# terry19850829Home/kafkastreams-cep

Hardware: AMD Instinct MI355X
Metric: events/sec (whole node), 3-stage A->B->C over 1M keys; achieved HBM GB/s (higher is better)
Workload: dtype int32; 1 GPU; C2: 3-stage strict A->B->C, processor mode; events_per_gpu=100000000, keys_per_gpu=1000000, matches_per_gpu=1531088, matches_total=1531088, parallelism=1 GPU, kernels=built-in, nfa_kernel=auto

## Files before the change

kafkastreams-cep_amd/csrc/abi.cpp:

```cpp
#include <dlfcn.h>
#include <hip/hip_runtime.h>
#include <string.h>

#include <algorithm>
#include <atomic>
#include <chrono>
#include <memory>
#include <string>
#include <vector>

#include "../../include/kcep.h"
#include "build_id.h"
#include "kcep_internal.h"
#include "jit.h"

namespace kcep {
hipError_t stencil_launch(const StencilLaunch& L, hipEvent_t ev0, hipEvent_t ev1, hipStream_t st);
int64_t stencil_tiles(int64_t n);
hipError_t stencil_post(const int32_t* key, const int32_t* out, int k, int64_t nm, int32_t* mkey,
                        const StencilProgram* P, unsigned long long* sum, hipStream_t st);
hipError_t stencil_resolve_launch(const int32_t* key, const int32_t* out, int k, int64_t nm, const StencilCarry& C,
                                  int64_t* pos, const StencilProgram* P, unsigned long long* sum, hipStream_t st);
hipError_t stencil_deliver_launch(const int32_t* key, const int32_t* out, int k, const int64_t* total, int64_t out_cap,
                                  const StencilCarry& C, int64_t host_cap, int64_t* hdr, int32_t* hkey, int64_t* hpos,
// ... 274 lines not shown
      if (arrs[i].src && arrs[i].bytes) {
        memcpy(h + at[size_t(i)], arrs[i].src, arrs[i].bytes);
        *arrs[i].dst = static_cast<uint8_t*>(dptr) + at[size_t(i)];
      }
    s->zc_slot = j;
    return CEP_OK;
  }
  bool pinned = true;
  for (int i = 0; i < na && pinned; i++)
    if (arrs[i].src && arrs[i].bytes) pinned = host_pinned(arrs[i].src);
  if (s->dstage.ensure(total)) return fail(CEP_E_HIP, "staging allocation failed");
  uint8_t* dev = s->dstage.as<uint8_t>();
  for (int i = 0; i < na; i++)
    if (arrs[i].src && arrs[i].bytes) *arrs[i].dst = dev + at[size_t(i)];
  if (pinned) {
    for (int i = 0; i < na; i++)
      if (arrs[i].src && arrs[i].bytes)
        HIPCHECK(hipMemcpyAsync(dev + at[size_t(i)], arrs[i].src, arrs[i].bytes, hipMemcpyHostToDevice, st));
    if (!s->h2d_ev) HIPCHECK(hipEventCreateWithFlags(&s->h2d_ev, hipEventDisableTiming));
    HIPCHECK(hipEventRecord(s->h2d_ev, st));
    s->h2d_wait = true;
    return CEP_OK;
  }
  const size_t chunk = std::min(total, size_t(2) << 20);
  for (size_t c0 = 0; c0 < total; c0 += chunk) {
    const size_t c1 = std::min(total, c0 + chunk);
    const int j = s->ring_next;
    s->ring_next ^= 1;
    if (s->ring_ev[j]) HIPCHECK(hipEventSynchronize(s->ring_ev[j]));
    else HIPCHECK(hipEventCreateWithFlags(&s->ring_ev[j], hipEventDisableTiming));
    const size_t want = std::min(total, chunk);
    if (s->ring_cap[j] < want) {
      if (s->ring[j]) HIPCHECK(hipHostFree(s->ring[j]));
      s->ring[j] = nullptr;
      s->ring_cap[j] = 0;
      HIPCHECK(hipHostMalloc(&s->ring[j], want, hipHostMallocMapped));
      s->ring_cap[j] = want;
    }
    uint8_t* h = static_cast<uint8_t*>(s->ring[j]);
    for (int i = 0; i < na; i++) {
      if (!arrs[i].src || !arrs[i].bytes) continue;
      const size_t a = std::max(c0, at[size_t(i)]), b = std::min(c1, at[size_t(i)] + arrs[i].bytes);
      if (a < b) memcpy(h + (a - c0), static_cast<const uint8_t*>(arrs[i].src) + (a - at[size_t(i)]), b - a);
    }
    HIPCHECK(hipMemcpyAsync(dev + c0, h, c1 - c0, hipMemcpyHostToDevice, st));
    HIPCHECK(hipEventRecord(s->ring_ev[j], st));
  }
  return CEP_OK;
}

void dl_layout(const cep_session* s, int slot, int64_t*& hdr, int32_t*& hkey, int64_t*& hpos) {
  hdr = static_cast<int64_t*>(s->dl[slot]);
  hkey = reinterpret_cast<int32_t*>(hdr + 4);
  hpos = hdr + 4 + (s->dl_cap + 1) / 2 + 1;
}

int push_stencil(cep_session* s, const cep_batch* b, hipStream_t st) {
  const StencilProgram& SP = s->pat->prog.stencil;
  const void* col = b->n_cols ? b->cols[SP.col] : nullptr;
  const int32_t* key = b->key_id;
  const int32_t* topic = SP.use_topic ? b->topic : nullptr;
  const size_t vs = type_size(SP.coltype);
  if (b->mem == CEP_MEM_HOST && b->n > 0) {
    HostArr arrs[3] = {{key, size_t(b->n) * 4, reinterpret_cast<const void**>(&key)},
                       {col, size_t(b->n) * vs, &col},
                       {topic, size_t(b->n) * 4, reinterpret_cast<const void**>(&topic)}};
    int rc = stage_host(s, arrs, SP.use_topic ? 3 : 2, st, true);
    if (rc) return rc;
  }
  if (SP.use_topic && !topic && b->n > 0) {
    if (s->h_topic.ensure(size_t(b->n) * 4)) return fail(CEP_E_HIP, "staging allocation failed");
    HIPCHECK(hipMemsetAsync(s->h_topic.p, 0, size_t(b->n) * 4, st));
    topic = s->h_topic.as<int32_t>();
  }
  if ((reinterpret_cast<uintptr_t>(key) | reinterpret_cast<uintptr_t>(col) | reinterpret_cast<uintptr_t>(topic)) & 15)
    return fail(CEP_E_ARG, "device columns must be 16-byte aligned");
  s->d_key = key;
  int64_t* tc = s->status.as<int64_t>();
  const int64_t ntiles = stencil_tiles(b->n);
  StencilLaunch L{key, col, topic, b->n, s->prog.as<StencilProgram>(), SP.k, SP.coltype, SP.use_topic, SP.chain,
                  s->slots.as<int32_t>(), tc, tc + ntiles + 1, s->counter.as<int64_t>(), s->out.as<int32_t>(),
                  s->out_cap, s->total.as<int64_t>(), StencilCarry{}, !getenv_flag("KCEP_STENCIL_KEYED"), nullptr};
  L.key_mode = getenv_flag("KCEP_STENCIL_SPARSE_KEYS") ? 1 : getenv_flag("KCEP_STENCIL_DENSE_KEYS") ? 2 : 0;
  if (s->carry) {
    L.clear_flag = s->hflags.as<unsigned long long>() + (s->halo_stamp & 1);
    L.carry = StencilCarry{s->halo.as<HaloHdr>(), s->hpos.as<int64_t>(), SP.k - 1, ++s->halo_stamp,
                           int32_t(std::min<int64_t>(s->opts.max_keys, INT32_MAX)), s->base,
                           s->hflags.as<unsigned long long>() + (s->halo_stamp & 1), s->cur_pos,
                           s->cur_pos ? 1 : 0};
    s->last_gpos = s->cur_pos;
    s->halo_base = s->base;
    s->base += b->n;
  }
  if (s->carry && (b->flags & CEP_BATCH_DELIVER)) {
    const int k = SP.k;
    const int64_t host_cap = std::min<int64_t>(s->out_cap, int64_t(1) << 20);
    if (!s->dl[0]) {
      const size_t bytes = 8 * (4 + size_t(host_cap + 1) / 2 + 1) + size_t(host_cap) * size_t(k) * 8;
      for (int j = 0; j < 2; j++) {
        HIPCHECK(hipHostMalloc(&s->dl[j], bytes, hipHostMallocMapped | hipHostMallocCoherent));
        memset(s->dl[j], 0, 32);
      }
      s->dl_cap = host_cap;
      if (s->dl_ticket.ensure(16)) return fail(CEP_E_HIP, "allocation failed");
      HIPCHECK(hipMemsetAsync(s->dl_ticket.p, 0, 16, st));
    }
    if (s->out_cap > host_cap &&
        (s->mkey.ensure(size_t(s->out_cap) * 4) || s->opos.ensure(size_t(s->out_cap) * size_t(k) * 8)))
      return fail(CEP_E_HIP, "allocation failed");
    const int slot = int((s->dl_stamp + 1) & 1);
    dl_layout(s, slot, L.deliver.hdr, L.deliver.hkey, L.deliver.hpos);
    s->dl_pid[slot] = s->push_id;
    L.deliver.dkey = s->mkey.as<int32_t>();
    L.deliver.dpos = s->opos.as<int64_t>();
    L.deliver.host_cap = s->dl_cap;
    L.deliver.ticket = s->dl_ticket.as<unsigned>();
    L.deliver.stamp = ++s->dl_stamp;
    if (s->cur_pos && b->n > 0) {
      if (s->a_moff.ensure(size_t(b->n) * 8) || s->a_tmp.ensure(size_t(b->n / 1024 + 4) * 8) || s->scal.ensure(64))
        return fail(CEP_E_HIP, "allocation failed");
      L.deliver.a_cnt = s->a_cnt.as<int64_t>();
      L.deliver.a_head = s->a_head.as<int32_t>();
      L.deliver.a_moff = s->a_moff.as<int64_t>();
      L.deliver.a_tot = s->scal.as<int64_t>() + 6;
      L.deliver.a_tmp = s->a_tmp.as<int64_t>();
      L.deliver.a_n = b->n;
    }
    s->delivered = true;
  }
  HIPCHECK(stencil_launch(L, s->timing ? s->ev0 : nullptr, s->timing ? s->ev1 : nullptr, st));
  if (s->timing) HIPCHECK(hipEventRecord(s->eb1, st));
  return CEP_OK;
}

int64_t read_i64(const void* dev, hipStream_t st, int* rc) {
  int64_t v = 0;
  if (hipMemcpyAsync(&v, dev, sizeof v, hipMemcpyDeviceToHost, st) != hipSuccess ||
      hipStreamSynchronize(st) != hipSuccess)
    *rc = CEP_E_HIP;
  return v;
}

int carry_gc(cep_session* s, int64_t min_words, hipStream_t st) {
  const int64_t nk = s->opts.max_keys;
  int rc = CEP_OK;
  if (s->flag.ensure(size_t(nk) * 8) || s->idx.ensure(size_t(nk) * 8) ||
      s->scan_tmp.ensure(size_t(nk / 1024 + 2) * 8) || s->scal.ensure(64))
    return fail(CEP_E_HIP, "allocation failed");
  int64_t* scal = s->scal.as<int64_t>();
  HIPCHECK(carry_sizes_launch(s->ctab.as<int64_t>(), nk, s->cpool.as<int32_t>(), s->flag.as<int64_t>(), st));
  HIPCHECK(exclusive_scan(s->flag.as<int64_t>(), nk, s->idx.as<int64_t>(), scal + 5, s->scan_tmp.as<int64_t>(), st));
  const int64_t live = read_i64(scal + 5, st, &rc);
  if (rc) return fail(rc, "carry size");
  const int64_t cap = std::max<int64_t>({2 * live, min_words, int64_t(1) << 20});
  DBuf fresh;
  if (fresh.ensure(size_t(cap) * 4)) return fail(CEP_E_RUN_CAPACITY, "cannot allocate the carried-state pool");
  HIPCHECK(carry_move_launch(s->ctab.as<int64_t>(), nk, s->cpool.as<int32_t>(), s->idx.as<int64_t>(),
                             fresh.as<int32_t>(), st));
  HIPCHECK(hipStreamSynchronize(st));
  s->cpool.release();
  s->cpool = fresh;
  fresh.p = nullptr;
  s->cpool_words = cap;
  s->cpool_used = live;
  return CEP_OK;
}
// ... 1924 lines not shown
```

kafkastreams-cep_amd/csrc/kcep_internal.h:

```cpp
#pragma once
#include <hip/hip_runtime_api.h>
#include <stdint.h>
#include "kcep_dev.h"

#include <memory>
#include <string>
#include <vector>

namespace kcep {

struct Expr {
  uint8_t op = 0, t = 0, ct = 0;
  int32_t i32 = 0;
  int64_t i64 = 0;
  double f64 = 0;
  int col = 0, name = 0;
  std::string sname;
  std::shared_ptr<Expr> a, b;
};
using ExprP = std::shared_ptr<Expr>;

struct Fold {
  int state;
  uint8_t type;
// ... 101 lines not shown
KCEP_HD inline int64_t halo_gpos(const StencilCarry& C, int64_t r) { return C.gpos ? C.gpos[r] : C.base + r; }
KCEP_HD inline int halo_old(const HaloHdr& h, int32_t stamp) {
  const int32_t a = h.stamp[0] < stamp ? h.stamp[0] : -1, b = h.stamp[1] < stamp ? h.stamp[1] : -1;
  return a >= b ? 0 : 1;
}

struct DeliverArgs {
  int64_t* hdr = nullptr;
  int32_t* hkey = nullptr;
  int64_t* hpos = nullptr;
  int32_t* dkey = nullptr;
  int64_t* dpos = nullptr;
  int64_t host_cap = 0;
  unsigned* ticket = nullptr;
  int64_t stamp = 0;
  int64_t* a_cnt = nullptr;
  int32_t* a_head = nullptr;
  int64_t* a_moff = nullptr;
  int64_t* a_tot = nullptr;
  int64_t* a_tmp = nullptr;
  int64_t a_n = 0;
};
struct GroupArgs {
  const int32_t* key;
  int32_t* g_key;
  int32_t* arr;
  int64_t* pos;
  int64_t base;
  const uint8_t* valid; uint8_t* g_valid;
  const int32_t* topic; int32_t* g_topic;
  const int32_t* partition; int32_t* g_partition;
  const int64_t* offset; int64_t* g_offset;
  const int64_t* ts; int64_t* g_ts;
  const void* cols[16]; void* g_cols[16];
  int32_t coltype[16];
  int32_t ncols;
  int64_t* cnt;
  int64_t* ecnt;
  int32_t max_keys;
  uint32_t stamp;
  unsigned long long* head;
  int32_t* node_top;
  int32_t *node_key, *node_chunk, *node_cnt, *node_next, *node_prefix, *node_leader, *rec_node, *rec_rank;
  int64_t* start;
  unsigned long long* cursor;
};
hipError_t group_launch(const GroupArgs& G, int64_t n, hipStream_t st);
hipError_t arrival_reorder(const int64_t* mrec, const int32_t* mkey, const int64_t* eoff, const int32_t* ename,
                           const int64_t* erec, int64_t nm, int64_t ne, int64_t base, int64_t n, int64_t* cnt,
                           int64_t* ecnt, int32_t* head, int64_t* moff, int64_t* moff_e, int64_t* tot, int64_t* tmp,
                           int64_t* o_rec, int32_t* o_key, int64_t* o_eoff, int32_t* o_name, int64_t* o_erec,
                           hipStream_t st);
hipError_t stencil_arrival_ranks(const int32_t* out, int k, const int64_t* total, int64_t out_cap, const int64_t* gpos,
                                 int64_t base, int64_t n, int64_t* cnt, int32_t* head, int64_t* moff, int64_t* tot,
                                 int64_t* tmp, hipStream_t st);
#ifndef KCEP_ST_DENSE
#define KCEP_ST_DENSE 512
#endif
constexpr int ST_DENSE = KCEP_ST_DENSE;
constexpr int ST_DENSE_KEYED = 1024;
#ifndef ST_KEYED_DENSE
#define ST_KEYED_DENSE 0
#endif

struct StencilLaunch {
  const int32_t* key;
  const void* val;
  const int32_t* topic;
  int64_t n;
  const StencilProgram* prog_dev;
  int k, coltype, use_topic, chain;
  int32_t* slots;
  int64_t* tile_count;
  int64_t* tile_pre;
  int64_t* scan_tmp;
  int32_t* out;
  int64_t out_cap;
  int64_t* total;
  StencilCarry carry;
  int plain;
  unsigned long long* clear_flag;
  DeliverArgs deliver;
  int key_mode = 0;
};

int lower_general(Program& P, std::string& why);
bool wave_stateful(const DevProgram& D);
int compile_ir(const uint8_t* ir, size_t len, Program& out, std::string& err);

struct RcIn {
  const int64_t* pos;
  const int32_t* key;
  const int32_t* topic;
  const int32_t* partition;
  const int64_t* offset;
  const int64_t* ts;
  const void* cols[16];
};
struct RcExt {
  int32_t *key, *topic, *partition, *seg;
  int64_t *offset, *ts, *pos;
  void* cols[16];
  int32_t coltype[16];
  int32_t ncols;
  int64_t cap;
};
hipError_t runs_carry_build(const RcIn& B, int64_t n, int64_t base, const int64_t* seg_flag, const int64_t* seg_idx,
                            const int64_t* seg_start, const int64_t* nseg, const int64_t* rtab, const int64_t* rpool,
                            int64_t* tlen, int64_t* toff, int64_t* total, int64_t* scan_tmp, const RcExt& X,
                            hipStream_t st, bool lens_only, int32_t max_keys);
hipError_t runs_carry_count(int64_t* out, int64_t nb, const int64_t* tails, int64_t cap, hipStream_t st);
hipError_t runs_carry_tails(const RcExt& X, int64_t ext_n, int64_t n, const int64_t* nseg, const int64_t* seg_start,
                            const int32_t* key, const int64_t* toff, const int32_t* end_of, unsigned long long* tstart,
                            int64_t* newlen, int64_t* noff, int64_t* new_total, int64_t* scan_tmp, int64_t* top,
                            int64_t* rpool, int64_t* rtab, hipStream_t st, const int64_t* ext_n_dev, const int64_t* bad);
hipError_t runs_carry_gc(int64_t* rtab, int64_t nkeys, int RW, const int64_t* src, int64_t* dst, int64_t* len,
                         int64_t* off, int64_t* total, int64_t* scan_tmp, hipStream_t st);

}
```

kafkastreams-cep_amd/csrc/stencil.hip:

```cpp
#include "stencil_kernel.h"

namespace kcep {

hipError_t stencil_count_k1(const StencilLaunch& L, hipStream_t st);
hipError_t stencil_count_k2(const StencilLaunch& L, hipStream_t st);
hipError_t stencil_count_k3(const StencilLaunch& L, hipStream_t st);
hipError_t stencil_count_k4(const StencilLaunch& L, hipStream_t st);
hipError_t stencil_count_k5(const StencilLaunch& L, hipStream_t st);
hipError_t stencil_count_k6(const StencilLaunch& L, hipStream_t st);
hipError_t stencil_count_k7(const StencilLaunch& L, hipStream_t st);
hipError_t stencil_count_k8(const StencilLaunch& L, hipStream_t st);

struct SlotFormat {
  int k, plain, chain, carry, dense, kdense;
  int64_t nsuper;
  int sub;
  __device__ __forceinline__ void load(const int32_t* slots, int64_t t, int64_t c, int64_t m, int32_t& v,
                                       uint32_t& a) const {
    a = 0;
    if (dense) {
      v = m < ST_DENSE ? slots[t * ST_DENSE + m] : slots[nsuper * ST_DENSE + t * int64_t(sub) * ST_TILE + m];
      return;
    }
    if (kdense && c <= ST_DENSE_KEYED) {
// ... 145 lines not shown
                                                  int64_t* __restrict__ total, unsigned long long* __restrict__ clear_flag) {
  __shared__ int64_t s_w[16];
  const int tid = threadIdx.x, lane = tid & 63, wid = tid >> 6;
  const int64_t per = (nt + 1023) / 1024, a = tid * per, b = a + per < nt ? a + per : nt;
  int64_t sum = 0;
  int64_t r8[8];
  const bool one_pass = per <= 8;
  if (one_pass) {
#pragma unroll
    for (int i = 0; i < 8; i++) { r8[i] = a + i < b ? cnt[a + i] : 0; sum += r8[i]; }
  } else {
    for (int64_t c = a; c < b; c += 8) {
      int64_t v[8];
#pragma unroll
      for (int i = 0; i < 8; i++) v[i] = c + i < b ? cnt[c + i] : 0;
#pragma unroll
      for (int i = 0; i < 8; i++) sum += v[i];
    }
  }
  int64_t incl = sum;
#pragma unroll
  for (int d = 1; d < 64; d <<= 1) {
    const int64_t y = __shfl_up(incl, d, 64);
    if (lane >= d) incl += y;
  }
  if (lane == 63) s_w[wid] = incl;
  __syncthreads();
  int64_t run = incl - sum;
  for (int w = 0; w < wid; w++) run += s_w[w];
  if (one_pass) {
#pragma unroll
    for (int i = 0; i < 8; i++)
      if (a + i < b) { pre[a + i] = run; run += r8[i]; }
  } else {
    for (int64_t c = a; c < b; c += 8) {
      int64_t v[8];
#pragma unroll
      for (int i = 0; i < 8; i++) v[i] = c + i < b ? cnt[c + i] : 0;
#pragma unroll
      for (int i = 0; i < 8; i++) {
        if (c + i < b) pre[c + i] = run;
        run += v[i];
      }
    }
  }
  if (tid == 1023) *total = run;
  if (tid == 0 && clear_flag) *clear_flag = 0;
}

constexpr int SMALL_FINISH = 1024;
__global__ __launch_bounds__(1024) void stencil_finish_small(const int32_t* __restrict__ slots,
                                                             const int64_t* __restrict__ cnt, int64_t nt, int k,
                                                             int32_t* __restrict__ out, int64_t out_cap, int sub,
                                                             int64_t* __restrict__ total,
                                                             unsigned long long* __restrict__ clear_flag,
                                                             SlotFormat F) {
  __shared__ int64_t s_pre[SMALL_FINISH + 1];
  __shared__ int64_t s_w[16];
  const int tid = threadIdx.x, lane = tid & 63, wid = tid >> 6;
  const int64_t c = tid < nt ? cnt[tid] : 0;
  int64_t incl = c;
#pragma unroll
  for (int d = 1; d < 64; d <<= 1) {
    const int64_t y = __shfl_up(incl, d, 64);
    if (lane >= d) incl += y;
  }
  if (lane == 63) s_w[wid] = incl;
  __syncthreads();
  int64_t run = incl - c;
  for (int w = 0; w < wid; w++) run += s_w[w];
  s_pre[tid] = run;
  if (tid == 1023) { s_pre[SMALL_FINISH] = run + c; *total = run + c; }
  if (tid == 0 && clear_flag) *clear_flag = 0;
  __syncthreads();
  for (int64_t t = wid; t < nt; t += 16) {
    const int64_t pre = s_pre[t], m = s_pre[t + 1] - pre;
    if (pre + m > out_cap) continue;
    int32_t* dst = out + pre * k;
    for (int64_t q = lane; q < m; q += 64) {
      int32_t v;
      uint32_t a;
      F.load(slots, t, m, q, v, a);
      for (int s2 = 0; s2 < k; s2++) dst[q * k + s2] = F.value(v, a, s2);
    }
  }
}

__device__ __forceinline__ void deliver_done(unsigned* ticket, unsigned nblocks, int64_t* hdr, int64_t stamp) {
  __syncthreads();
  if (threadIdx.x == 0) {
    __threadfence_system();
    const unsigned prev = atomicAdd(ticket, 1u);
    if (prev == nblocks - 1) {
      __threadfence_system();
      *ticket = 0;
      *reinterpret_cast<volatile int64_t*>(hdr + 2) = stamp;
    }
  }
}

__global__ __launch_bounds__(256) void stencil_finish_deliver(const int32_t* __restrict__ slots,
                                                              const int64_t* __restrict__ cnt, int64_t nt, int k,
                                                              int32_t* __restrict__ out, int64_t out_cap, int sub,
                                                              int64_t* __restrict__ total,
                                                              unsigned long long* __restrict__ clear_flag,
                                                              SlotFormat F, const int32_t* __restrict__ key,
                                                              StencilCarry C, int64_t host_cap, int64_t* __restrict__ hdr,
                                                              int32_t* __restrict__ hkey, int64_t* __restrict__ hpos,
                                                              int32_t* __restrict__ dkey, int64_t* __restrict__ dpos,
                                                              unsigned* ticket, int64_t stamp) {
  __shared__ int64_t s_red[2][4];
  const int64_t t = blockIdx.x;
  const int lane = threadIdx.x & 63, wid = threadIdx.x >> 6;
  int64_t before = 0, all = 0;
  for (int64_t i = threadIdx.x; i < nt; i += 256) {
    const int64_t c = cnt[i];
    all += c;
    if (i < t) before += c;
  }
#pragma unroll
  for (int d = 32; d >= 1; d >>= 1) {
    before += __shfl_xor(before, d, 64);
    all += __shfl_xor(all, d, 64);
  }
  if (lane == 0) { s_red[0][wid] = before; s_red[1][wid] = all; }
  __syncthreads();
  const int64_t pre = s_red[0][0] + s_red[0][1] + s_red[0][2] + s_red[0][3];
  const int64_t tot = s_red[1][0] + s_red[1][1] + s_red[1][2] + s_red[1][3];
  if (t == 0 && threadIdx.x == 0) {
    *total = tot;
    hdr[0] = tot;
    hdr[1] = int64_t(*C.flags);
    if (clear_flag) *clear_flag = 0;
  }
  const int64_t m = cnt[t];
  if (pre + m <= out_cap) {
    for (int64_t q = threadIdx.x; q < m; q += 256) {
      const int64_t i = pre + q;
      int32_t row[STENCIL_MAX_K], last = 0, v;
      uint32_t av;
      F.load(slots, t, m, q, v, av);
#pragma unroll
      for (int s = 0; s < STENCIL_MAX_K; s++)
        if (s < k) {
          row[s] = F.value(v, av, s);
          out[i * k + s] = row[s];
          last = row[s];
        }
      const int32_t kk = key[last];
      const bool kok = kk >= 0 && kk < C.max_keys;
      const HaloHdr* h = kok ? C.hdr + kk : nullptr;
      const int old = kok ? halo_old(*h, C.stamp) : 0;
      const int64_t* hp = kok ? C.pos + (2 * int64_t(kk) + old) * C.km1 : nullptr;
      const bool host = i < host_cap;
      int64_t* p = host ? hpos + i * k : dpos + i * k;
#pragma unroll
      for (int s = 0; s < STENCIL_MAX_K; s++)
        if (s < k) {
          const int32_t r = row[s];
          p[s] = r >= 0 ? halo_gpos(C, r) : (r == -1 || !kok ? -1 : hp[h->cnt[old] - (-r - 1)]);
        }
      if (host) hkey[i] = kk;
      else dkey[i] = kk;
    }
  }
  deliver_done(ticket, unsigned(gridDim.x), hdr, stamp);
// ... 105 lines not shown
      int64_t j = s_tpre[a >> 6];
      for (int64_t b = (a & ~int64_t(63)) >> 2; b < (a >> 2); b++) {
        const uint32_t w = s_cnt[b];
        j += (w & 0xFF) + ((w >> 8) & 0xFF) + ((w >> 16) & 0xFF) + (w >> 24);
      }
      for (int64_t b = a & ~int64_t(3); b < a; b++) j += (s_cnt[b >> 2] >> (8 * (b & 3))) & 0xFF;
      if (F.chain)
        for (int64_t p = q - 1; p >= 0 && F.entry(slots, t, m, p, k - 1) == last; p--) j++;
      const bool kok = kk >= 0 && kk < C.max_keys;
      const HaloHdr* h = kok ? C.hdr + kk : nullptr;
      const int old = kok ? halo_old(*h, C.stamp) : 0;
      const int64_t* hp = kok ? C.pos + (2 * int64_t(kk) + old) * C.km1 : nullptr;
      const bool host = j < host_cap;
      int64_t* pp = host ? hpos + j * k : dpos + j * k;
#pragma unroll
      for (int s2 = 0; s2 < STENCIL_MAX_K; s2++)
        if (s2 < k) {
          const int32_t r = row[s2];
          pp[s2] = r >= 0 ? halo_gpos(C, r) : (r == -1 || !kok ? -1 : hp[h->cnt[old] - (-r - 1)]);
        }
      if (host) hkey[j] = kk;
      else dkey[j] = kk;
    }
  }
  (void)n;
  deliver_done(ticket, 1u, hdr, stamp);
}

static hipError_t stencil_count(const StencilLaunch& L, hipStream_t st) {
  if (L.chain && L.k != 3 && L.k != 4) return hipErrorInvalidValue;
  switch (L.k) {
    case 1: return stencil_count_k1(L, st);
    case 2: return stencil_count_k2(L, st);
    case 3: return stencil_count_k3(L, st);
    case 4: return stencil_count_k4(L, st);
    case 5: return stencil_count_k5(L, st);
    case 6: return stencil_count_k6(L, st);
    case 7: return stencil_count_k7(L, st);
    case 8: return stencil_count_k8(L, st);
  }
  return hipErrorInvalidValue;
}

hipError_t exclusive_scan(const int64_t* in, int64_t n, int64_t* out, int64_t* total, int64_t* tmp, hipStream_t st);
hipError_t stencil_deliver_launch(const int32_t* key, const int32_t* out, int k, const int64_t* total, int64_t out_cap,
                                  const StencilCarry& C, const DeliverArgs& D, hipStream_t st);

hipError_t stencil_launch(const StencilLaunch& L, hipEvent_t ev0, hipEvent_t ev1, hipStream_t st) {
  const DeliverArgs& D = L.deliver;
  if (L.n <= 0) {
    hipError_t e = ev0 ? hipEventRecord(ev0, st) : hipSuccess;
    if (e == hipSuccess && L.clear_flag) e = hipMemsetAsync(L.clear_flag, 0, 8, st);
    if (e == hipSuccess && ev1) e = hipEventRecord(ev1, st);
    if (e == hipSuccess) e = hipMemsetAsync(L.total, 0, sizeof(int64_t), st);
    if (e == hipSuccess && D.hdr)
      e = stencil_deliver_launch(L.key, L.out, L.k, L.total, 0, L.carry, D, st);
    return e;
  }
  const int64_t ntiles = (L.n + ST_TILE - 1) / ST_TILE;
  const int sub = stencil_sub(ntiles);
  const int64_t nsuper = (ntiles + sub - 1) / sub;
  hipError_t e = ev0 ? hipEventRecord(ev0, st) : hipSuccess;
  if (e == hipSuccess) e = stencil_count(L, st);
  if (e == hipSuccess && ev1) e = hipEventRecord(ev1, st);
  if (e != hipSuccess) return e;
  const bool plain = L.plain && !L.chain && L.k <= 7;
  const SlotFormat F{L.k, plain, L.chain, L.carry.hdr != nullptr, plain && !L.carry.hdr && ST_PLAIN_STAGE,
                     !plain && !L.carry.hdr && ST_KEYED_DENSE, nsuper, sub};
  if (nsuper <= SMALL_FINISH && D.hdr && L.carry.hdr && D.a_moff && L.n <= ARR_SMALL) {
    hipLaunchKernelGGL(stencil_finish_deliver_arrival, dim3(1), dim3(1024), 0, st, L.slots, L.tile_count, nsuper, L.k,
                       L.out, L.out_cap, sub, L.total, L.clear_flag, F, L.key, L.carry, L.n, D.host_cap, D.hdr, D.hkey,
                       D.hpos, D.dkey, D.dpos, D.ticket, D.stamp);
    return hipGetLastError();
  }
  if (nsuper <= SMALL_FINISH && D.hdr && L.carry.hdr && !D.a_moff) {
    hipLaunchKernelGGL(stencil_finish_deliver, dim3(unsigned(nsuper)), dim3(256), 0, st, L.slots, L.tile_count, nsuper,
                       L.k, L.out, L.out_cap, sub, L.total, L.clear_flag, F, L.key, L.carry, D.host_cap, D.hdr, D.hkey,
                       D.hpos, D.dkey, D.dpos, D.ticket, D.stamp);
    return hipGetLastError();
  }
  if (nsuper <= SMALL_FINISH) {
    hipLaunchKernelGGL(stencil_finish_small, dim3(1), dim3(1024), 0, st, L.slots, L.tile_count, nsuper, L.k, L.out,
                       L.out_cap, sub, L.total, L.clear_flag, F);
  } else {
    if (nsuper <= 8 * 1024) {
      hipLaunchKernelGGL(tile_scan, dim3(1), dim3(1024), 0, st, L.tile_count, nsuper, L.tile_pre, L.total, L.clear_flag);
    } else {
      hipError_t e = exclusive_scan(L.tile_count, nsuper, L.tile_pre, L.total, L.scan_tmp, st);
      if (e == hipSuccess && L.clear_flag) e = hipMemsetAsync(L.clear_flag, 0, 8, st);
      if (e != hipSuccess) return e;
    }
    if (F.dense) {
      decltype(&stencil_gather_dense<1>) g = nullptr;
      switch (L.k) {
        case 1: g = stencil_gather_dense<1>; break;
        case 2: g = stencil_gather_dense<2>; break;
        case 3: g = stencil_gather_dense<3>; break;
        case 4: g = stencil_gather_dense<4>; break;
        case 5: g = stencil_gather_dense<5>; break;
        case 6: g = stencil_gather_dense<6>; break;
        case 7: g = stencil_gather_dense<7>; break;
        default: return hipErrorInvalidValue;
      }
      hipLaunchKernelGGL(g, dim3(unsigned(nsuper)), dim3(128), 0, st, L.slots, L.tile_count, L.tile_pre, L.out,
                         L.out_cap, nsuper, sub);
    } else {
      decltype(&stencil_gather_k<1>) g = nullptr;
      switch (L.k) {
        case 1: g = stencil_gather_k<1>; break;
        case 2: g = stencil_gather_k<2>; break;
        case 3: g = stencil_gather_k<3>; break;
        case 4: g = stencil_gather_k<4>; break;
        case 5: g = stencil_gather_k<5>; break;
        case 6: g = stencil_gather_k<6>; break;
        case 7: g = stencil_gather_k<7>; break;
        case 8: g = stencil_gather_k<8>; break;
        default: break;
      }
      if (g) {
        hipLaunchKernelGGL(g, dim3(unsigned(nsuper)), dim3(128), 0, st, L.slots, L.tile_count, L.tile_pre, L.out,
                           L.out_cap, F);
      } else {
        hipLaunchKernelGGL(stencil_gather, dim3(unsigned(nsuper)), dim3(128), 0, st, L.slots, L.tile_count, L.tile_pre,
                           L.out, L.out_cap, sub, F);
      }
    }
  }
  if (D.hdr) {
    hipError_t e = hipGetLastError();
    if (e != hipSuccess) return e;
    return stencil_deliver_launch(L.key, L.out, L.k, L.total, L.out_cap, L.carry, D, st);
  }
  return hipGetLastError();
}

__global__ void stencil_gather_keys(const int32_t* __restrict__ key, const int32_t* __restrict__ out, int k,
                                    int64_t nm, int32_t* __restrict__ mkey) {
  const int64_t i = int64_t(blockIdx.x) * blockDim.x + threadIdx.x;
  if (i < nm) mkey[i] = key[out[i * k + k - 1]];
}

__device__ __forceinline__ uint64_t mix64(uint64_t x) {
  x ^= x >> 33; x *= 0xff51afd7ed558ccdULL; x ^= x >> 33; x *= 0xc4ceb9fe1a85ec53ULL; x ^= x >> 33;
  return x;
}

__global__ void stencil_checksum(const int32_t* __restrict__ out, int k, int64_t nm,
                                 const StencilProgram* __restrict__ P, unsigned long long* __restrict__ sum) {
  const int64_t i = int64_t(blockIdx.x) * blockDim.x + threadIdx.x;
  uint64_t h = 0;
  if (i < nm) {
    const int64_t j = out[i * k + k - 1];
    h = mix64(uint64_t(j) * 0x9e3779b97f4a7c15ULL);
    for (int s = k - 1; s >= 0; s--) {
      const int32_t r = out[i * k + s];
      if (r >= 0) h = mix64(h ^ (uint64_t(r) << 8) ^ uint64_t(P->name[s]));
    }
  }
  for (int d = 32; d >= 1; d >>= 1) h += __shfl_xor(h, d, 64);
  if ((threadIdx.x & 63) == 0 && h) atomicAdd(sum, (unsigned long long)h);
}

__global__ void stencil_resolve(const int32_t* __restrict__ key, const int32_t* __restrict__ out, int k, int64_t nm,
                                StencilCarry C, int64_t* __restrict__ pos) {
  const int64_t i = int64_t(blockIdx.x) * blockDim.x + threadIdx.x;
  if (i >= nm) return;
// ... 92 lines not shown
```

kafkastreams-cep_amd/csrc/stencil_kernel.h:

```cpp
#pragma once
#include <hip/hip_runtime.h>
#include <stdint.h>

#include <type_traits>

#include "kcep_internal.h"

namespace kcep {

constexpr int ST_THREADS = 256;
constexpr int ST_EPT = 16;
constexpr int ST_TILE = ST_THREADS * ST_EPT;
constexpr int ST_SUB = 4;
inline int stencil_sub(int64_t ntiles) { return ntiles >= int64_t(ST_SUB) * 2048 ? ST_SUB : 1; }

typedef int v4i __attribute__((ext_vector_type(4)));
typedef long long v2l __attribute__((ext_vector_type(2)));
__device__ __forceinline__ v4i ld_nt4(const void* p) { return __builtin_nontemporal_load(reinterpret_cast<const v4i*>(p)); }
__device__ __forceinline__ v2l ld_nt2(const void* p) { return __builtin_nontemporal_load(reinterpret_cast<const v2l*>(p)); }

__device__ __forceinline__ int kpos(int rp) { return rp + 4 * (rp >> 4); }
constexpr int ST_KWORDS = (ST_TILE + 16) + 4 * ((ST_TILE + 16) >> 4) + 16;

template <class VT>
// ... 657 lines not shown
      c.v[q].a = ld_nt4(vb + o);
    } else {
      c.v[q].a = ld_nt2(vb + o);
      c.v[q].b = ld_nt2(vb + o + 2);
    }
    if constexpr (TOPIC) c.t[q] = ld_nt4(tb + o);
  }
}

#ifndef ST_PLAIN_DENSE_LANES
#define ST_PLAIN_DENSE_LANES 40
#endif
constexpr int ST_KEYS_ADAPTIVE = 0, ST_KEYS_SPARSE = 1, ST_KEYS_DENSE = 2;
template <int K>
__device__ __forceinline__ uint32_t window_same_keys(const int32_t* __restrict__ key, int64_t g0, int64_t n,
                                                     uint32_t cand, int mode, int lane) {
  const uint64_t holders = __ballot(cand != 0);
  if (holders == 0) return 0;
  const bool dense = mode == ST_KEYS_DENSE || (mode == ST_KEYS_ADAPTIVE && __popcll(holders) > ST_PLAIN_DENSE_LANES);
  int32_t k[ST_EPT], pk[K - 1];
#pragma unroll
  for (int i = 0; i < ST_EPT; i++) k[i] = 0;
#pragma unroll
  for (int t = 0; t < K - 1; t++) pk[t] = 0;
  auto own = [&](bool nt) {
    if (g0 + ST_EPT <= n) {
#pragma unroll
      for (int q = 0; q < ST_EPT / 4; q++) {
        const v4i v = nt ? ld_nt4(key + g0 + 4 * q) : *reinterpret_cast<const v4i*>(key + g0 + 4 * q);
        k[4 * q] = v[0]; k[4 * q + 1] = v[1]; k[4 * q + 2] = v[2]; k[4 * q + 3] = v[3];
      }
    } else {
#pragma unroll
      for (int i = 0; i < ST_EPT; i++) k[i] = key[g0 + i < n ? g0 + i : n - 1];
    }
  };
  auto before = [&]() {
#pragma unroll
    for (int t = 0; t < K - 1; t++) {
      const int64_t g = g0 - (K - 1) + t;
      pk[t] = key[g < 0 ? 0 : g < n ? g : n - 1];
    }
  };
  if (dense) {
    own(true);
#pragma unroll
    for (int t = 0; t < K - 1; t++)
      pk[t] = __builtin_amdgcn_update_dpp(0, k[ST_EPT - (K - 1) + t], 0x138, 0xF, 0xF, false);
    if (lane == 0) before();
  } else {
    if (cand != 0) own(false);
    if (cand & ((1u << (K - 1)) - 1u)) before();
  }
  uint32_t S = uint32_t(k[0] == pk[K - 2]) << 8;
#pragma unroll
  for (int i = 1; i < ST_EPT; i++) S |= uint32_t(k[i] == k[i - 1]) << (8 + i);
#pragma unroll
  for (int t = 1; t < K - 1; t++) S |= uint32_t(pk[t] == pk[t - 1]) << (8 - (K - 1) + t);
  return S;
}

#ifndef ST_PLAIN_EARLY
#define ST_PLAIN_EARLY 1
#endif
#ifndef ST_PLAIN_WAVES
#define ST_PLAIN_WAVES 6
#endif
#ifndef ST_PLAIN_STAGE
#define ST_PLAIN_STAGE 1
#endif
#ifndef ST_PLAIN_NTSTORE
#define ST_PLAIN_NTSTORE 1
#endif
#ifndef ST_PLAIN_PROBE
#define ST_PLAIN_PROBE 0
#endif
#ifndef ST_CARRY_WAVES
#define ST_CARRY_WAVES 4
#endif
template <int K, class VT, bool TOPIC, int SUB, bool CARRY>
__global__ __launch_bounds__(ST_THREADS, CARRY ? ST_CARRY_WAVES : ST_PLAIN_WAVES) void stencil_plain_kernel(
    const int32_t* __restrict__ key, const VT* __restrict__ val, const int32_t* __restrict__ topic, int64_t n,
    const StencilProgram* __restrict__ P, int32_t* __restrict__ out, int64_t* __restrict__ tile_count,
    int64_t ntiles, StencilCarry C, int key_mode) {
  static_assert(K >= 1 && K <= 7, "bit 7 of a record's byte is its same-key bit");
  __shared__ __attribute__((aligned(16))) uint8_t s_mask[ST_TILE + 16];
  __shared__ int32_t s_bk[CARRY ? ST_TILE + 16 : 1];
  __shared__ int32_t s_lastk[CARRY ? 2 : 1][CARRY ? 17 : 1];
  __shared__ int32_t s_firstk[CARRY ? 16 : 1];
  __shared__ int32_t s_wsum[2][ST_THREADS / 64];
  __shared__ uint8_t s_tab[64];
  __shared__ uint8_t s_lut[256];
  __shared__ uint8_t s_nan[4];
  constexpr bool STAGE = !CARRY && ST_PLAIN_STAGE;
  __shared__ int32_t s_out[STAGE ? ST_TILE : 1];

  const int tid = threadIdx.x;
  const int lane = tid & 63, wid = tid >> 6;
  if (tid < 64) s_tab[tid] = P->table[tid];
  s_lut[tid] = P->lut[tid];
  if (tid < 4) s_nan[tid] = P->nan_mask[tid];
  const int64_t tile0 = int64_t(blockIdx.x) * SUB;
  const int ntl = int(ntiles - tile0 < SUB ? ntiles - tile0 : SUB);

  Chunk<VT, TOPIC> cur;
  load_tile<VT, TOPIC, CARRY>(cur, key, val, topic, tile0 * ST_TILE, n, tid);
  const bool halo_lane = tid >= 16 - (K - 1) && tid < 16;
  const int64_t hg = tile0 * ST_TILE - 16 + tid;
  int32_t h_key = INT32_MIN, h_prev = INT32_MIN, h_top = 0;
  VT h_val{};
  if (halo_lane && hg >= 0) {
    h_val = val[hg];
    if constexpr (TOPIC) h_top = topic[hg];
    if constexpr (CARRY) {
      h_key = key[hg];
      if (hg > 0) h_prev = key[hg - 1];
    }
  }
  int32_t before0 = INT32_MIN;
  if constexpr (CARRY)
    if (tid == 0 && tile0 > 0) before0 = key[tile0 * ST_TILE - 1];
  __syncthreads();
  uint32_t h_mask = 0;
  if (halo_lane && hg >= 0)
    h_mask = mask_of<VT, TOPIC>(P, s_tab, s_nan, h_val, h_top) | (uint32_t(CARRY && hg > 0 && h_prev == h_key) << 7);
  int32_t h_bk = h_key;
  bool twice = false;

  int32_t* slot = out + tile0 * int64_t(ST_TILE) * K;
  uint8_t* const aux = reinterpret_cast<uint8_t*>(slot + SUB * ST_TILE);
  int64_t sum = 0;
  int nbuf = 0;
  int32_t* const dense = out + int64_t(blockIdx.x) * ST_DENSE;
  int32_t* const over = out + int64_t(gridDim.x) * ST_DENSE + tile0 * ST_TILE;
  for (int j = 0; j < ntl; j++) {
    const int64_t base = (tile0 + j) * ST_TILE;
    int32_t nk = INT32_MIN;
    if constexpr (CARRY)
      if (tid == ST_THREADS - 1 && base + ST_TILE < n) nk = key[base + ST_TILE];
    uint32_t packed[4];
    masks_of_chunk<VT, TOPIC>(cur, P, s_tab, s_nan, packed, s_lut);
#pragma unroll
    for (int q = 0; q < ST_EPT / 4; q++) {
      const int local = q * (ST_THREADS * 4) + tid * 4;
      uint32_t w = packed[q];
      const int64_t left = n - (base + local);
      if constexpr (CARRY) {
        const v4i k = cur.k[q];
        const int32_t kp = __builtin_amdgcn_update_dpp(INT32_MIN, k[3], 0x138, 0xF, 0xF, false);
        const uint32_t same = uint32_t(lane > 0 && kp == k[0]) | (uint32_t(k[1] == k[0]) << 8) |
                              (uint32_t(k[2] == k[1]) << 16) | (uint32_t(k[3] == k[2]) << 24);
        w |= same << 7;
        if (lane == 0) s_firstk[4 * q + wid] = k[0];
        if (lane == 63) s_lastk[j & 1][4 * q + wid + 1] = k[3];
        const int32_t kn = __builtin_amdgcn_update_dpp(INT32_MIN, k[0], 0x130, 0xF, 0xF, false);
        const bool c1 = k[1] != k[0] || left <= 1, c2 = k[2] != k[1] || left <= 2, c3 = k[3] != k[2] || left <= 3;
        if (lane == 0 || kp != k[0] || c1) s_bk[16 + local] = k[0];
        if (c1 || c2) s_bk[16 + local + 1] = k[1];
        if (c2 || c3) s_bk[16 + local + 2] = k[2];
        if (c3 || lane == 63 || kn != k[3] || left <= 4) s_bk[16 + local + 3] = k[3];
      }
      if (left < 4) w &= left <= 0 ? 0u : (0xFFFFFFFFu >> (8 * (4 - left)));
      *reinterpret_cast<uint32_t*>(&s_mask[16 + local]) = w;
    }
    if (tid < 16) s_mask[tid] = halo_lane ? uint8_t(h_mask) : 0;
    if constexpr (CARRY)
      if (tid < 16) s_bk[tid] = h_bk;
    if constexpr (CARRY)
// ... 132 lines not shown
        int32_t* ws = out + tile0 * int64_t(ST_TILE) * K + j * ST_TILE + wid * 1024 + before;
        const int32_t b32 = int32_t(base) - (K - 1);
        while (hit) {
          const int i = __ffs(hit) - 1;
          hit &= hit - 1;
          *ws++ = b32 + tid * ST_EPT + i;
        }
      }
      sum += wtot;
      continue;
    }
#endif
    if (lane == 0) s_wsum[j & 1][wid] = wtot;
    if (halo_lane) h_mask = s_mask[ST_TILE + tid];
    if constexpr (CARRY)
      if (halo_lane) h_bk = s_bk[ST_TILE + tid];
    __syncthreads();
    int o = before, tot = 0;
#pragma unroll
    for (int w = 0; w < ST_THREADS / 64; w++) {
      const int x = s_wsum[j & 1][w];
      o += w < wid ? x : 0;
      tot += x;
    }
    tot = __builtin_amdgcn_readfirstlane(tot);
    const int32_t b32 = int32_t(base) - (K - 1);
    if constexpr (STAGE) {
      const int p0 = int(sum) + o;
      if (ST_PLAIN_PROBE == 3) {
        sum += tot;
        continue;
      }
      if (sum + tot <= ST_TILE) {
        for (int q = 0; hit; q++) {
          const int i = __ffs(hit) - 1;
          hit &= hit - 1;
          s_out[p0 + q] = b32 + tid * ST_EPT + i;
        }
        nbuf = int(sum) + tot;
      } else {
        for (int q = 0; hit; q++) {
          const int i = __ffs(hit) - 1;
          hit &= hit - 1;
          const int p = p0 + q;
          (p < ST_DENSE ? dense : over)[p] = b32 + tid * ST_EPT + i;
        }
      }
      sum += tot;
      continue;
    }
    while (hit) {
      const int i = __ffs(hit) - 1;
      hit &= hit - 1;
      if constexpr (CARRY) {
        const uint32_t need = uint32_t(bneed >> (4 * i)) & 0xFu;
        if (need) {
          slot[o] = -(1 + int32_t(base) + tid * ST_EPT + i);
          aux[sum + o] = uint8_t(need);
          o++;
          continue;
        }
      }
      slot[o++] = b32 + tid * ST_EPT + i;
    }
    slot += tot;
    sum += tot;
  }
  if constexpr (STAGE) {
    __syncthreads();
#if ST_PLAIN_NTSTORE
    for (int i = tid; i < nbuf; i += ST_THREADS) __builtin_nontemporal_store(s_out[i], &(i < ST_DENSE ? dense : over)[i]);
#else
    for (int i = tid; i < nbuf; i += ST_THREADS) (i < ST_DENSE ? dense : over)[i] = s_out[i];
#endif
  }
#if ST_PLAIN_PROBE == 1 || ST_PLAIN_PROBE == 2
  if constexpr (!CARRY) {
    if (lane == 0) s_wsum[0][wid] = int(sum);
    __syncthreads();
    if (tid == 0) tile_count[blockIdx.x] = s_wsum[0][0] + s_wsum[0][1] + s_wsum[0][2] + s_wsum[0][3];
    return;
  }
#endif
  if (tid == 0) tile_count[blockIdx.x] = sum;
  if constexpr (CARRY)
    if (twice) atomicOr(C.flags, 2ull);
}

template <int K, class VT, bool TP, bool CH, int SUB>
inline void launch_kts(const StencilLaunch& L, int64_t ntiles, hipStream_t st) {
  const int64_t nsuper = (ntiles + SUB - 1) / SUB;
  if constexpr (!CH && K <= 7) {
    if (L.plain) {
      if (L.carry.hdr)
        hipLaunchKernelGGL((stencil_plain_kernel<K, VT, TP, SUB, true>), dim3(unsigned(nsuper)), dim3(ST_THREADS), 0, st,
                           L.key, static_cast<const VT*>(L.val), L.topic, L.n, L.prog_dev, L.slots, L.tile_count,
                           ntiles, L.carry, L.key_mode);
      else
        hipLaunchKernelGGL((stencil_plain_kernel<K, VT, TP, SUB, false>), dim3(unsigned(nsuper)), dim3(ST_THREADS), 0, st,
                           L.key, static_cast<const VT*>(L.val), L.topic, L.n, L.prog_dev, L.slots, L.tile_count,
                           ntiles, L.carry, L.key_mode);
      return;
    }
  }
  if (L.carry.hdr)
    hipLaunchKernelGGL((stencil_kernel<K, VT, TP, CH, true, SUB>), dim3(unsigned(nsuper)), dim3(ST_THREADS), 0, st,
                       L.key, static_cast<const VT*>(L.val), L.topic, L.n, L.prog_dev, L.slots, L.tile_count, ntiles,
                       L.carry);
  else
    hipLaunchKernelGGL((stencil_kernel<K, VT, TP, CH, false, SUB>), dim3(unsigned(nsuper)), dim3(ST_THREADS), 0, st,
                       L.key, static_cast<const VT*>(L.val), L.topic, L.n, L.prog_dev, L.slots, L.tile_count, ntiles,
                       L.carry);
}

template <int K, class VT, bool TP, bool CH>
inline hipError_t launch_kt(const StencilLaunch& L, hipStream_t st) {
  const int64_t ntiles = (L.n + ST_TILE - 1) / ST_TILE;
  if (stencil_sub(ntiles) == ST_SUB) launch_kts<K, VT, TP, CH, ST_SUB>(L, ntiles, st);
  else launch_kts<K, VT, TP, CH, 1>(L, ntiles, st);
  return hipGetLastError();
}

template <int K, bool CH = false>
inline hipError_t launch_k(const StencilLaunch& L, hipStream_t st) {
  if (L.coltype == T_I32)
    return L.use_topic ? launch_kt<K, int32_t, true, CH>(L, st) : launch_kt<K, int32_t, false, CH>(L, st);
  if (L.coltype == T_I64)
    return L.use_topic ? launch_kt<K, int64_t, true, CH>(L, st) : launch_kt<K, int64_t, false, CH>(L, st);
  return L.use_topic ? launch_kt<K, double, true, CH>(L, st) : launch_kt<K, double, false, CH>(L, st);
}

}
```

Before: 1000 billion events/s.

## Fuse tile scan and dense finish into one kernel using 16-bit counts

Adds a stencil_finish_dense kernel in which each block computes its own prefix offset by redundantly summing packed 16-bit super-tile counts, then writes its matches directly. This replaces the separate single-block tile_scan followed by the finish launch. The plain kernel now also writes a 16-bit copy of each count into the tile_pre buffer so the prefix reads are compact and vectorised. The cost is redundant prefix work in every block. It also relies on the tile_pre area being free for the 16-bit counts and does not clear clear_flag on this path.

```diff
diff --git a/kafkastreams-cep_amd/csrc/abi.cpp b/kafkastreams-cep_amd/csrc/abi.cpp
--- a/kafkastreams-cep_amd/csrc/abi.cpp
+++ b/kafkastreams-cep_amd/csrc/abi.cpp
@@ -380,6 +380,8 @@
                   s->slots.as<int32_t>(), tc, tc + ntiles + 1, s->counter.as<int64_t>(), s->out.as<int32_t>(),
                   s->out_cap, s->total.as<int64_t>(), StencilCarry{}, !getenv_flag("KCEP_STENCIL_KEYED"), nullptr};
   L.key_mode = getenv_flag("KCEP_STENCIL_SPARSE_KEYS") ? 1 : getenv_flag("KCEP_STENCIL_DENSE_KEYS") ? 2 : 0;
+  L.tile_count16 = reinterpret_cast<uint16_t*>((reinterpret_cast<uintptr_t>(L.tile_pre) + 15) & ~uintptr_t(15));
+  L.split_finish = getenv_flag("KCEP_STENCIL_SPLIT_FINISH");
   if (s->carry) {
     L.clear_flag = s->hflags.as<unsigned long long>() + (s->halo_stamp & 1);
     L.carry = StencilCarry{s->halo.as<HaloHdr>(), s->hpos.as<int64_t>(), SP.k - 1, ++s->halo_stamp,
diff --git a/kafkastreams-cep_amd/csrc/kcep_internal.h b/kafkastreams-cep_amd/csrc/kcep_internal.h
--- a/kafkastreams-cep_amd/csrc/kcep_internal.h
+++ b/kafkastreams-cep_amd/csrc/kcep_internal.h
@@ -207,6 +207,8 @@
   unsigned long long* clear_flag;
   DeliverArgs deliver;
   int key_mode = 0;
+  uint16_t* tile_count16 = nullptr;
+  int split_finish = 0;
 };
 
 int lower_general(Program& P, std::string& why);
diff --git a/kafkastreams-cep_amd/csrc/stencil.hip b/kafkastreams-cep_amd/csrc/stencil.hip
--- a/kafkastreams-cep_amd/csrc/stencil.hip
+++ b/kafkastreams-cep_amd/csrc/stencil.hip
@@ -251,6 +251,108 @@
       uint32_t a;
       F.load(slots, t, m, q, v, a);
       for (int s2 = 0; s2 < k; s2++) dst[q * k + s2] = F.value(v, a, s2);
+    }
+  }
+}
+
+#ifndef FIN_G
+#define FIN_G 4
+#endif
+#ifndef FIN_WPS
+#define FIN_WPS 1
+#endif
+#ifndef FIN_B
+#define FIN_B 5
+#endif
+constexpr int FIN_U = 4;
+constexpr int FIN_THREADS = FIN_G * FIN_WPS * 64;
+constexpr int FIN_MAX_SUPER = 8 * 1024;
+constexpr int FIN_ROUNDS = (FIN_MAX_SUPER / 8 + FIN_THREADS - 1) / FIN_THREADS;
+static_assert(FIN_THREADS <= 1024 && FIN_B * 64 * FIN_WPS <= ST_DENSE, "the first round stays inside the dense region");
+static_assert(int64_t(FIN_MAX_SUPER) * ST_SUB * ST_TILE < (int64_t(1) << 31), "32-bit partial sums of the counts");
+typedef unsigned v4u __attribute__((ext_vector_type(4)));
+template <int K>
+__global__ __launch_bounds__(FIN_THREADS) void stencil_finish_dense(const int32_t* __restrict__ slots,
+                                                                    const uint16_t* __restrict__ cnt16,
+                                                                    int32_t* __restrict__ out, int64_t out_cap, int nsuper,
+                                                                    int sub, int64_t* __restrict__ total) {
+  __shared__ int32_t s_w[FIN_THREADS / 64];
+  const int tid = threadIdx.x, lane = tid & 63, wid = tid >> 6;
+  const int t0 = int(blockIdx.x) * FIN_G;
+  const int g = wid / FIN_WPS, part = wid % FIN_WPS;
+  const int t = t0 + g;
+  const int tc = t < nsuper ? t : nsuper - 1;
+  const int32_t* const dense = slots + int64_t(tc) * ST_DENSE;
+  int32_t v[FIN_B];
+#pragma unroll
+  for (int q = 0; q < FIN_B; q++) v[q] = dense[(q * FIN_WPS + part) * 64 + lane];
+  const int nfull = nsuper >> 3;
+  v4u cv[FIN_ROUNDS];
+#pragma unroll
+  for (int r = 0; r < FIN_ROUNDS; r++) {
+    const int i = r * FIN_THREADS + tid;
+    cv[r] = *reinterpret_cast<const v4u*>(cnt16 + 8 * (i < nfull ? i : nfull - 1));
+  }
+  const int ti = 8 * nfull + (tid & 7);
+  const int tail = cnt16[ti < nsuper ? ti : nsuper - 1];
+  const int oi = t0 + (lane < FIN_G ? lane : 0);
+  const int own = cnt16[oi < nsuper ? oi : nsuper - 1];
+  int before = 0;
+#pragma unroll
+  for (int r = 0; r < FIN_ROUNDS; r++) {
+    const int i = r * FIN_THREADS + tid;
+    const int nb = i < nfull ? t0 - 8 * i : 0;
+    if (nb >= 8) {
+#pragma unroll
+      for (int w = 0; w < 4; w++) before += int(cv[r][w] & 0xFFFFu) + int(cv[r][w] >> 16);
+    } else if (nb > 0) {
+#pragma unroll
+      for (int w = 0; w < 4; w++)
+        before += (2 * w < nb ? int(cv[r][w] & 0xFFFFu) : 0) + (2 * w + 1 < nb ? int(cv[r][w] >> 16) : 0);
+    }
+  }
+  if (tid < 8 && ti < t0) before += tail;
+#pragma unroll
+  for (int d = 32; d >= 1; d >>= 1) before += __shfl_xor(before, d, 64);
+  if (lane == 0) s_w[wid] = before;
+  __syncthreads();
+  int64_t p = 0;
+#pragma unroll
+  for (int w = 0; w < FIN_THREADS / 64; w++) p += s_w[w];
+  int c = 0, csum = 0;
+#pragma unroll
+  for (int i = 0; i < FIN_G; i++) {
+    const int ci = t0 + i < nsuper ? __builtin_amdgcn_readlane(own, i) : 0;
+    p += i < g ? ci : 0;
+    c = i == g ? ci : c;
+    csum += ci;
+  }
+  if (t0 + FIN_G >= nsuper && tid == 0) *total = p + csum;
+  if (p + c > out_cap || c <= 0) return;
+  int32_t* const dst = out + p * K;
+#pragma unroll
+  for (int q = 0; q < FIN_B; q++) {
+    const int m = (q * FIN_WPS + part) * 64 + lane;
+    if (m < c) {
+#pragma unroll
+      for (int s = 0; s < K; s++) dst[int64_t(m) * K + s] = v[q] + s;
+    }
+  }
+  const int32_t* const over = slots + int64_t(nsuper) * ST_DENSE + int64_t(t) * sub * ST_TILE;
+  for (int m0 = FIN_B * FIN_WPS * 64; m0 < c; m0 += FIN_U * FIN_WPS * 64) {
+    int32_t w[FIN_U];
+#pragma unroll
+    for (int u = 0; u < FIN_U; u++) {
+      const int m = m0 + (u * FIN_WPS + part) * 64 + lane, mm = m < c ? m : c - 1;
+      w[u] = (mm < ST_DENSE ? dense : over)[mm];
+    }
+#pragma unroll
+    for (int u = 0; u < FIN_U; u++) {
+      const int m = m0 + (u * FIN_WPS + part) * 64 + lane;
+      if (m < c) {
+#pragma unroll
+        for (int s = 0; s < K; s++) dst[int64_t(m) * K + s] = w[u] + s;
+      }
     }
   }
 }
@@ -522,6 +624,20 @@
   if (nsuper <= SMALL_FINISH) {
     hipLaunchKernelGGL(stencil_finish_small, dim3(1), dim3(1024), 0, st, L.slots, L.tile_count, nsuper, L.k, L.out,
                        L.out_cap, sub, L.total, L.clear_flag, F);
+  } else if (F.dense && nsuper <= FIN_MAX_SUPER && !L.split_finish) {
+    decltype(&stencil_finish_dense<1>) f = nullptr;
+    switch (L.k) {
+      case 1: f = stencil_finish_dense<1>; break;
+      case 2: f = stencil_finish_dense<2>; break;
+      case 3: f = stencil_finish_dense<3>; break;
+      case 4: f = stencil_finish_dense<4>; break;
+      case 5: f = stencil_finish_dense<5>; break;
+      case 6: f = stencil_finish_dense<6>; break;
+      case 7: f = stencil_finish_dense<7>; break;
+      default: return hipErrorInvalidValue;
+    }
+    hipLaunchKernelGGL(f, dim3(unsigned((nsuper + FIN_G - 1) / FIN_G)), dim3(FIN_THREADS), 0, st, L.slots,
+                       L.tile_count16, L.out, L.out_cap, int(nsuper), sub, L.total);
   } else {
     if (nsuper <= 8 * 1024) {
       hipLaunchKernelGGL(tile_scan, dim3(1), dim3(1024), 0, st, L.tile_count, nsuper, L.tile_pre, L.total, L.clear_flag);
diff --git a/kafkastreams-cep_amd/csrc/stencil_kernel.h b/kafkastreams-cep_amd/csrc/stencil_kernel.h
--- a/kafkastreams-cep_amd/csrc/stencil_kernel.h
+++ b/kafkastreams-cep_amd/csrc/stencil_kernel.h
@@ -763,8 +763,9 @@
 __global__ __launch_bounds__(ST_THREADS, CARRY ? ST_CARRY_WAVES : ST_PLAIN_WAVES) void stencil_plain_kernel(
     const int32_t* __restrict__ key, const VT* __restrict__ val, const int32_t* __restrict__ topic, int64_t n,
     const StencilProgram* __restrict__ P, int32_t* __restrict__ out, int64_t* __restrict__ tile_count,
-    int64_t ntiles, StencilCarry C, int key_mode) {
+    int64_t ntiles, StencilCarry C, int key_mode, uint16_t* __restrict__ tile_count16) {
   static_assert(K >= 1 && K <= 7, "bit 7 of a record's byte is its same-key bit");
+  static_assert(ST_SUB * ST_TILE <= 0xFFFF, "a super-tile's match count is also stored as a 16-bit word");
   __shared__ __attribute__((aligned(16))) uint8_t s_mask[ST_TILE + 16];
   __shared__ int32_t s_bk[CARRY ? ST_TILE + 16 : 1];
   __shared__ int32_t s_lastk[CARRY ? 2 : 1][CARRY ? 17 : 1];
@@ -1063,7 +1064,10 @@
     return;
   }
 #endif
-  if (tid == 0) tile_count[blockIdx.x] = sum;
+  if (tid == 0) {
+    tile_count[blockIdx.x] = sum;
+    if constexpr (!CARRY) tile_count16[blockIdx.x] = uint16_t(sum);
+  }
   if constexpr (CARRY)
     if (twice) atomicOr(C.flags, 2ull);
 }
@@ -1076,11 +1080,11 @@
       if (L.carry.hdr)
         hipLaunchKernelGGL((stencil_plain_kernel<K, VT, TP, SUB, true>), dim3(unsigned(nsuper)), dim3(ST_THREADS), 0, st,
                            L.key, static_cast<const VT*>(L.val), L.topic, L.n, L.prog_dev, L.slots, L.tile_count,
-                           ntiles, L.carry, L.key_mode);
+                           ntiles, L.carry, L.key_mode, L.tile_count16);
       else
         hipLaunchKernelGGL((stencil_plain_kernel<K, VT, TP, SUB, false>), dim3(unsigned(nsuper)), dim3(ST_THREADS), 0, st,
                            L.key, static_cast<const VT*>(L.val), L.topic, L.n, L.prog_dev, L.slots, L.tile_count,
-                           ntiles, L.carry, L.key_mode);
+                           ntiles, L.carry, L.key_mode, L.tile_count16);
       return;
     }
   }
```

Measured after the change: 1056 billion events/s, median of 6. +5.6%, better.
